# SebastianBitsch/SRGAN-ST

Measured on AMD Instinct MI355X. Metric: HR images/sec (96px x4, B=16/GPU) G+D+ST-loss step, higher is better.
Workload: dtype f32; 1 GPU; srgan_x4_hr96_b16_G+D+ST-loss step: adv+mse+st, D updated every step (train.py:116-164; BASELINE metric); global_batch=16, hr=96, lr=24, parallelism=dp1, hip_graph=True, d_update_interval=1, d_sr_forward=run: all three discriminator forwards of train.py:136,155,158

## Files before the change

### include/srganst.h

```cpp
#ifndef SRGANST_H
#define SRGANST_H
#include <stdint.h>
#ifdef __cplusplus
extern "C" {
#endif

const char* sst_last_error(void);
int sst_version(void);
const char* sst_arch(void);
int sst_clear_error(void);
int sst_reload_env(void);

int sst_st_loss_workspace(int B, int H, int W, int64_t* partial_floats);
int sst_st_loss_fwd(const float* sr, const float* gt, float* loss, float* gS, float* partials,
                    unsigned* counter, int B, int H, int W, float sigma, float rho, int normalize,
                    void* stream);
int sst_st_loss_bwd(const float* sr, const float* gS, float* dsr, const float* scale_dev,
                    float scale_host, int accumulate, int B, int H, int W, float sigma, float rho,
                    void* stream);
int sst_st_maps_workspace(int B, int H, int W, int64_t* tile_floats);
int sst_st_maps(const float* x, const float* gt, float* Sx, float* Sgt, float* Fx, float* Fgt, float* d, float* tile_sums,
                int B, int H, int W, float sigma, float rho, int normalize, void* stream);
int sst_st_pixel_loss_fwd(const float* sr, const float* gt, float* loss, float* gS, float* partials, unsigned* counter,
                          float* pix_loss, float* pix_partials, int pix_mode, int B, int H, int W, float sigma, float rho,
// ... 182 lines not shown
int sst_pixel_loss_fwd(const float* x, const float* gt, float* loss, float* partials, unsigned* counter,
                       int64_t n, int mode, void* stream);
int sst_pixel_loss_bwd(const float* x, const float* gt, float* dx, const float* scale_dev,
                       float scale_host, int accumulate, int64_t n, int mode, void* stream);
int sst_bce_logits(const float* logits, float target, float* loss, float* dlogits,
                   const float* scale_dev, float scale_host, int n, void* stream);
int sst_bicubic(const float* x, float* y, const float* wy, const int* iy, const float* wx, const int* ix,
                int64_t planes, int H, int W, int oh, int ow, int Ty, int Tx, int round_grid, void* stream);
int sst_gather_batch(const uint8_t* src, int64_t N, const int* idx, int B, int H, int W, const float* lut, float* gt, float* lr,
                     const float* wy, const int* iy, const float* wx, const int* ix, int oh, int ow, int Ty, int Tx,
                     void* stream);
int sst_gather_crops(const uint8_t* arena, int64_t arena_bytes, const int64_t* table, int64_t N, const int* desc, int B, int S,
                     const float* lut, float* gt, float* lr, const float* wy, const int* iy, const float* wx, const int* ix,
                     int oh, int ow, int Ty, int Tx, int span, void* stream);
int sst_image_metrics_workspace(int B, int H, int W, int64_t* partial_doubles);
int sst_image_metrics(const float* sr, const float* hr, int B, int H, int W, double* out, uint8_t* sr_u8, uint8_t* hr_u8,
                      double* workspace, void* stream);
int sst_tile_gather(const uint8_t* src_u8, const float* src_f32, int64_t src_bytes, int H, int W, const int* desc, int B, int th,
                    int tw, int t, const float* lut, float* out, void* stream);
int sst_tile_scatter(const float* tiles, const int* rows, int B, int H, int W, int th, int tw, int scale, int t, float* canvas,
                     int accumulate, void* stream);
int sst_canvas_to_u8(const float* canvas, int H, int W, float scale, uint8_t* out, void* stream);
int sst_bb_blocks(int B, int H, int W);
int sst_bb_feature_dim(int mode);
int sst_bb_patches(const float* img, float* cand, float* cnrm, int B, int H, int W, int ncand_total, int cand_off,
                   int mode, const float* st_mats, void* stream);
int sst_bb_match(const float* sr, const float* cand, const float* cnrm, int* ind, float* dsr, float* partials, int B,
                 int H, int W, int ncand, float alpha, float beta, int criterion_l2, int mode, const float* st_mats,
                 void* stream);
int sst_bb_match_dist(const float* sr, const float* cand, const float* cnrm, int* ind, float* dsr, float* partials, int B,
                 int H, int W, int ncand, float alpha, float beta, int criterion_l2, int mode, const float* st_mats, int dist_l1,
                      void* stream);
int sst_bbg_patches(int H, int W, int k, int pad, int stride);
int sst_bbg_blocks(int B, int np);
int sst_bbg_unfold(const float* img, float* table, float* nrm, int B, int H, int W, int k, int pad, int stride, int nrows_total,
                   int row_off, void* stream);
int sst_bbg_match(const float* srf, const float* cand, const float* cnrm, int* ind, float* gfeat, float* partials, int B, int np,
                  int ncand, int D, float alpha, float beta, int criterion_l2, int dist_l1, void* stream);
int sst_bbg_fold(const float* gfeat, float* dsr, int B, int H, int W, int k, int pad, int stride, void* stream);
int sst_weighted_sum(const float* const* terms, const float* weights, int n, float* out, float* weighted,
                     void* stream);

int sst_linear_ksplit(int M, int N, int K);
int sst_linear_fwd(const float* x, const float* w, const float* bias, float* y, float* slab, int M, int N,
                   int K, void* stream);
int sst_linear_dgrad(const float* dy, const float* w, float* dx, int M, int N, int K, int nhwc_C,
                     int nhwc_HW, void* stream);
int sst_linear_wgrad(const float* dy, const float* x, float* dw, float* db, int M, int N, int K,
                     int accumulate, void* stream);
int sst_head_fwd(const float* h, const float* w, const float* b, float* y, int M, int N, int K, float slope,
                 void* stream);
int sst_head_bwd(const float* h, const float* w, const float* dy, float* dh, float* dw, float* db, int M,
                 int N, int K, float slope, int accumulate, void* stream);
int sst_flatten_act(const float* y, const float* scale, const float* shift, float slope, int act,
                    float* flat, int B, int HW, int C, void* stream);
int sst_flatten_act_grp(const float* y, const float* scale, const float* shift, float slope, int act,
                        float* flat, int B, int HW, int C, int grp_images, void* stream);

int sst_adam_flat(float* p, const float* g, float* m, float* v, int64_t n, const float* lr, float* steps,
                  int nsteps, double beta1, double beta2, double eps, double weight_decay, void* stream);

#ifdef __cplusplus
}
#endif
#endif
```

### srgan-st_amd/csrc/linear.hip

```cpp
#include "common.h"

typedef float f32x4 __attribute__((ext_vector_type(4)));

namespace {
constexpr int NT = 256;
constexpr int MAXM = 64;

__global__ __launch_bounds__(NT) void linear_fwd_kernel(const float* __restrict__ x, const float* __restrict__ w,
                                                        float* __restrict__ slab, int M, int N, int K, int kslice) {
  __shared__ float red[4][MAXM][17];
  const int wave = __builtin_amdgcn_readfirstlane(threadIdx.x >> 6), lane = threadIdx.x & 63;
  const int lj = lane & 15, lq = lane >> 4;
  const int n0 = blockIdx.x * 16;
  const int kb = blockIdx.y * kslice, ke = min(K, kb + kslice);
  const int mt = (M + 15) / 16;
  f32x4 acc[4];
#pragma unroll
  for (int t = 0; t < 4; ++t) acc[t] = f32x4{0.f, 0.f, 0.f, 0.f};
  const int n = min(n0 + lj, N - 1);
  const float* wrow = w + (size_t)n * K;
  for (int k = kb + wave * 16; k < ke; k += 64) {
    const int kk = k + 4 * lq;
    f32x4 bv = {0.f, 0.f, 0.f, 0.f};
    if (kk + 3 < ke) {
      bv = *reinterpret_cast<const f32x4*>(wrow + kk);
    } else {
#pragma unroll
      for (int j = 0; j < 4; ++j)
        if (kk + j < ke) bv[j] = wrow[kk + j];
    }
#pragma unroll
    for (int t = 0; t < 4; ++t) {
      if (t < mt) {
        const int m = t * 16 + lj;
        f32x4 av = {0.f, 0.f, 0.f, 0.f};
        if (m < M) {
          if (kk + 3 < ke) {
            av = *reinterpret_cast<const f32x4*>(x + (size_t)m * K + kk);
          } else {
#pragma unroll
            for (int j = 0; j < 4; ++j)
              if (kk + j < ke) av[j] = x[(size_t)m * K + kk + j];
          }
        }
#pragma unroll
        for (int j = 0; j < 4; ++j) acc[t] = __builtin_amdgcn_mfma_f32_16x16x4f32(av[j], bv[j], acc[t], 0, 0, 0);
      }
    }
  }
#pragma unroll
  for (int t = 0; t < 4; ++t)
#pragma unroll
    for (int r = 0; r < 4; ++r) red[wave][t * 16 + 4 * lq + r][lj] = acc[t][r];
  __syncthreads();
  for (int i = threadIdx.x; i < M * 16; i += NT) {
    const int m = i >> 4, j = i & 15;
    if (n0 + j < N)
      slab[((size_t)blockIdx.y * M + m) * N + n0 + j] = red[0][m][j] + red[1][m][j] + red[2][m][j] + red[3][m][j];
  }
}

__global__ __launch_bounds__(NT) void linear_reduce_kernel(const float* __restrict__ slab, const float* __restrict__ bias,
                                                           float* __restrict__ y, int nslab, int M, int N) {
  const int total = M * N;
  for (int i = blockIdx.x * NT + threadIdx.x; i < total; i += gridDim.x * NT) {
    float t = bias ? bias[i % N] : 0.f;
    for (int s = 0; s < nslab; ++s) t += slab[(size_t)s * total + i];
    y[i] = t;
  }
}

template <int MT>
__global__ __launch_bounds__(NT) void linear_dgrad_kernel(const float* __restrict__ dy, const float* __restrict__ w,
                                                          float* __restrict__ dx, int M, int N, int K, int C, int HW) {
  __shared__ float red[4][16][65];
  const int wave = __builtin_amdgcn_readfirstlane(threadIdx.x >> 6), lane = threadIdx.x & 63;
  const int lj = lane & 15, lq = lane >> 4;
  const int k0 = blockIdx.x * 64;
  const int nper = ((N + 3) / 4 + 3) / 4 * 4;
  const int nb = wave * nper, ne = min(N, nb + nper);
  f32x4 acc[MT][4];
#pragma unroll
  for (int mt = 0; mt < MT; ++mt)
#pragma unroll
    for (int t = 0; t < 4; ++t) acc[mt][t] = f32x4{0.f, 0.f, 0.f, 0.f};
  int n = nb;
  if (k0 + 64 <= K) {
    constexpr int U = MT == 1 ? 8 : 4;
    const float* wcol = w + k0 + 4 * lj;
    for (; n + 4 * U <= ne; n += 4 * U) {
      f32x4 bv[U];
      float av[MT][U];
#pragma unroll
      for (int u = 0; u < U; ++u) {
        const int nn = n + 4 * u + lq;
        bv[u] = *reinterpret_cast<const f32x4*>(wcol + (size_t)nn * K);
#pragma unroll
        for (int mt = 0; mt < MT; ++mt) {
          const int m = mt * 16 + lj;
          av[mt][u] = m < M ? dy[(size_t)m * N + nn] : 0.f;
        }
      }
#pragma unroll
      for (int u = 0; u < U; ++u)
#pragma unroll
        for (int mt = 0; mt < MT; ++mt)
#pragma unroll
          for (int t = 0; t < 4; ++t) acc[mt][t] = __builtin_amdgcn_mfma_f32_16x16x4f32(av[mt][u], bv[u][t], acc[mt][t], 0, 0, 0);
    }
  }
  for (; n < ne; n += 4) {
    const int nn = n + lq;
    f32x4 bv = {0.f, 0.f, 0.f, 0.f};
    if (nn < ne) {
      const int kk = k0 + 4 * lj;
      if (kk + 3 < K) {
        bv = *reinterpret_cast<const f32x4*>(w + (size_t)nn * K + kk);
      } else {
#pragma unroll
        for (int j = 0; j < 4; ++j)
          if (kk + j < K) bv[j] = w[(size_t)nn * K + kk + j];
      }
    }
#pragma unroll
    for (int mt = 0; mt < MT; ++mt) {
      const int m = mt * 16 + lj;
      const float av = (nn < ne && m < M) ? dy[(size_t)m * N + nn] : 0.f;
#pragma unroll
      for (int t = 0; t < 4; ++t) acc[mt][t] = __builtin_amdgcn_mfma_f32_16x16x4f32(av, bv[t], acc[mt][t], 0, 0, 0);
    }
  }
#pragma unroll
  for (int mt = 0; mt < MT; ++mt) {
    __syncthreads();
#pragma unroll
    for (int t = 0; t < 4; ++t)
#pragma unroll
      for (int r = 0; r < 4; ++r) red[wave][4 * lq + r][4 * lj + t] = acc[mt][t][r];
    __syncthreads();
    for (int i = threadIdx.x; i < 16 * 64; i += NT) {
      const int mm = i >> 6, kc = i & 63, mg = mt * 16 + mm, k = k0 + kc;
      if (mg < M && k < K) {
        const float v = red[0][mm][kc] + red[1][mm][kc] + red[2][mm][kc] + red[3][mm][kc];
        const size_t o = HW > 0 ? (size_t)mg * K + (size_t)(k % HW) * C + k / HW : (size_t)mg * K + k;
        dx[o] = v;
      }
    }
  }
}

__global__ __launch_bounds__(NT) void linear_wgrad_kernel(const float* __restrict__ dy, const float* __restrict__ x,
                                                          float* __restrict__ dw, int M, int N, int K, int accumulate) {
  __shared__ float sdy[MAXM][16];
  const int n0 = blockIdx.y * 16;
  for (int i = threadIdx.x; i < M * 16; i += NT) {
    const int m = i >> 4, j = i & 15;
    sdy[m][j] = (n0 + j < N) ? dy[(size_t)m * N + n0 + j] : 0.f;
  }
  __syncthreads();
  const int k = (blockIdx.x * NT + threadIdx.x) * 4;
  if (k >= K) return;
  const bool vec = (K & 3) == 0;
  f32x4 acc[16];
#pragma unroll
  for (int j = 0; j < 16; ++j) acc[j] = f32x4{0.f, 0.f, 0.f, 0.f};
  for (int m = 0; m < M; ++m) {
    f32x4 xv = {0.f, 0.f, 0.f, 0.f};
    if (vec) {
      xv = *reinterpret_cast<const f32x4*>(x + (size_t)m * K + k);
    } else {
#pragma unroll
      for (int j = 0; j < 4; ++j)
        if (k + j < K) xv[j] = x[(size_t)m * K + k + j];
    }
#pragma unroll
    for (int j = 0; j < 16; ++j) acc[j] += sdy[m][j] * xv;
  }
#pragma unroll
  for (int j = 0; j < 16; ++j) {
    if (n0 + j >= N) break;
// ... 108 lines not shown
#pragma unroll
          for (int i = 0; i < HB_ROWS; ++i) v[i] = mb + i < M ? h[(size_t)(mb + i) * K + k] : 0.f;
#pragma unroll
          for (int i = 0; i < HB_ROWS; ++i) {
            if (mb + i >= M) break;
            const float x = v[i] > 0.f ? v[i] : v[i] * slope;
            a = fmaf(dy[(size_t)(mb + i) * N + n], x, a);
          }
        }
        dw[(size_t)n * K + k] = accumulate ? dw[(size_t)n * K + k] + a : a;
      }
    }
  }
  if (db && blockIdx.x == 0 && blockIdx.y == 0 && threadIdx.x < N) {
    float t = 0.f;
    for (int m = 0; m < M; ++m) t += dy[(size_t)m * N + threadIdx.x];
    db[threadIdx.x] = accumulate ? db[threadIdx.x] + t : t;
  }
}

__global__ __launch_bounds__(NT) void flatten_act_kernel(const float* __restrict__ y, const float* __restrict__ scale,
                                                         const float* __restrict__ shift, float slope, int act,
                                                         float* __restrict__ flat, int B, int HW, int C, int gB) {
  const int64_t total = (int64_t)B * HW * C;
  for (int64_t i = blockIdx.x * (int64_t)NT + threadIdx.x; i < total; i += (int64_t)gridDim.x * NT) {
    const int c = (int)(i % C);
    const int64_t p = i / C;
    const int hw = (int)(p % HW);
    const int64_t b = p / HW;
    float v = y[i];
    if (scale) {
      const int gc = (int)(b / gB) * C + c;
      v = fmaf(v, scale[gc], shift[gc]);
    }
    if (act) v = v > 0.f ? v : v * slope;
    flat[(b * C + c) * HW + hw] = v;
  }
}
}

SST_API int sst_linear_ksplit(int M, int N, int K) {
  int ks = 1024 / ((N + 15) / 16);
  if (ks < 1) ks = 1;
  while (ks > 1 && K / ks < 256) ks >>= 1;
  return ks;
}

SST_API int sst_linear_fwd(const float* x, const float* w, const float* bias, float* y, float* slab, int M, int N, int K,
                           void* stream) {
  SST_REQUIRE(x && w && y && slab && M > 0 && M <= MAXM && N > 0 && K > 0, "sst_linear_fwd: bad argument (M=%d)", M);
  const int ks = sst_linear_ksplit(M, N, K);
  const int kslice = ((K + ks - 1) / ks + 63) / 64 * 64;
  dim3 grid((N + 15) / 16, (K + kslice - 1) / kslice);
  linear_fwd_kernel<<<grid, NT, 0, sst_stream(stream)>>>(x, w, slab, M, N, K, kslice);
  SST_LAUNCH_CHECK("linear_fwd_kernel");
  const int rb = (M * N + NT - 1) / NT;
  linear_reduce_kernel<<<rb < 512 ? rb : 512, NT, 0, sst_stream(stream)>>>(slab, bias, y, grid.y, M, N);
  SST_LAUNCH_CHECK("linear_reduce_kernel");
  return SST_OK;
}

SST_API int sst_linear_dgrad(const float* dy, const float* w, float* dx, int M, int N, int K, int nhwc_C, int nhwc_HW,
                             void* stream) {
  SST_REQUIRE(dy && w && dx && M > 0 && M <= MAXM && N > 0 && K > 0, "sst_linear_dgrad: bad argument");
  SST_REQUIRE(nhwc_HW == 0 || nhwc_C * nhwc_HW == K, "sst_linear_dgrad: C*HW must equal K");
  const int grid = (K + 63) / 64;
  hipStream_t st = sst_stream(stream);
  switch ((M + 15) / 16) {
    case 1: linear_dgrad_kernel<1><<<grid, NT, 0, st>>>(dy, w, dx, M, N, K, nhwc_C, nhwc_HW); break;
    case 2: linear_dgrad_kernel<2><<<grid, NT, 0, st>>>(dy, w, dx, M, N, K, nhwc_C, nhwc_HW); break;
    case 3: linear_dgrad_kernel<3><<<grid, NT, 0, st>>>(dy, w, dx, M, N, K, nhwc_C, nhwc_HW); break;
    default: linear_dgrad_kernel<4><<<grid, NT, 0, st>>>(dy, w, dx, M, N, K, nhwc_C, nhwc_HW); break;
  }
  SST_LAUNCH_CHECK("linear_dgrad_kernel");
  return SST_OK;
}

SST_API int sst_linear_wgrad(const float* dy, const float* x, float* dw, float* db, int M, int N, int K, int accumulate,
                             void* stream) {
  SST_REQUIRE(dy && x && dw && M > 0 && M <= MAXM && N > 0 && K > 0, "sst_linear_wgrad: bad argument");
  if ((K & 31) == 0 && (N & 63) == 0 && !sst_env("SST_LINEAR_WGRAD_FMA")) {
    linear_wgrad_mfma_kernel<<<dim3((K / 32 + 3) / 4, N / 64), NT, 0, sst_stream(stream)>>>(dy, x, dw, M, N, K, accumulate);
    SST_LAUNCH_CHECK("linear_wgrad_mfma_kernel");
  } else {
    dim3 grid((K + 4 * NT - 1) / (4 * NT), (N + 15) / 16);
    linear_wgrad_kernel<<<grid, NT, 0, sst_stream(stream)>>>(dy, x, dw, M, N, K, accumulate);
    SST_LAUNCH_CHECK("linear_wgrad_kernel");
  }
  if (db) {
    colsum_small_kernel<<<(N + 255) / 256, 256, 0, sst_stream(stream)>>>(dy, db, M, N, accumulate);
    SST_LAUNCH_CHECK("colsum_small_kernel");
  }
  return SST_OK;
}

SST_API int sst_head_fwd(const float* h, const float* w, const float* b, float* y, int M, int N, int K, float slope,
                         void* stream) {
  SST_REQUIRE(h && w && y && M > 0 && N > 0 && N <= 64 && K > 0, "sst_head_fwd: bad argument");
  head_fwd_kernel<<<M * N, NT, 0, sst_stream(stream)>>>(h, w, b, y, M, N, K, slope);
  SST_LAUNCH_CHECK("head_fwd_kernel");
  return SST_OK;
}

SST_API int sst_head_bwd(const float* h, const float* w, const float* dy, float* dh, float* dw, float* db, int M, int N,
                         int K, float slope, int accumulate, void* stream) {
  SST_REQUIRE(h && w && dy && dh && M > 0 && N > 0 && N <= 64 && K > 0, "sst_head_bwd: bad argument");
  head_bwd_kernel<<<dim3((K + NT - 1) / NT, (M + HB_ROWS - 1) / HB_ROWS), NT, 0, sst_stream(stream)>>>(h, w, dy, dh, dw, db, M, N, K, slope,
                                                                                                    accumulate);
  SST_LAUNCH_CHECK("head_bwd_kernel");
  return SST_OK;
}

SST_API int sst_flatten_act_grp(const float* y, const float* scale, const float* shift, float slope, int act, float* flat,
                                int B, int HW, int C, int grp_images, void* stream) {
  SST_REQUIRE(y && flat && B > 0 && HW > 0 && C > 0 && ((scale == nullptr) == (shift == nullptr)), "sst_flatten_act: bad argument");
  SST_REQUIRE(grp_images >= 0 && (grp_images == 0 || B % grp_images == 0), "sst_flatten_act: bad group size %d for B=%d", grp_images, B);
  const int64_t total = (int64_t)B * HW * C;
  const int blocks = (int)((total + NT - 1) / NT < 2048 ? (total + NT - 1) / NT : 2048);
  flatten_act_kernel<<<blocks, NT, 0, sst_stream(stream)>>>(y, scale, shift, slope, act, flat, B, HW, C, grp_images > 0 ? grp_images : B);
  SST_LAUNCH_CHECK("flatten_act_kernel");
  return SST_OK;
}
SST_API int sst_flatten_act(const float* y, const float* scale, const float* shift, float slope, int act, float* flat,
                            int B, int HW, int C, void* stream) {
  return sst_flatten_act_grp(y, scale, shift, slope, act, flat, B, HW, C, 0, stream);
}
// ... 1 lines not shown
```

### srgan-st_amd/srganst/_abi.py

```python
from __future__ import annotations

import ctypes
import os
from ctypes import c_char_p, c_float, c_int, c_int64, c_void_p, POINTER

_HERE = os.path.dirname(os.path.abspath(__file__))
LIB_PATH = os.environ.get("SST_LIB_PATH") or os.path.join(_HERE, "lib", "libsrganst.so")

P = c_void_p

SIGNATURES = {
    "sst_last_error": (c_char_p, []),
    "sst_version": (c_int, []),
    "sst_arch": (c_char_p, []),
    "sst_clear_error": (c_int, []),
    "sst_reload_env": (c_int, []),
    "sst_st_loss_workspace": (c_int, [c_int, c_int, c_int, POINTER(c_int64)]),
    "sst_st_loss_fwd": (c_int, [P, P, P, P, P, P, c_int, c_int, c_int, c_float, c_float, c_int, P]),
    "sst_st_loss_bwd": (c_int, [P, P, P, P, c_float, c_int, c_int, c_int, c_int, c_float, c_float, P]),
    "sst_st_pixel_loss_fwd": (c_int, [P, P, P, P, P, P, P, P, c_int, c_int, c_int, c_int, c_float, c_float, c_int, P]),
    "sst_st_pixel_loss_bwd": (c_int, [P, P, P, P, P, c_float, c_float, c_int, c_int, c_int, c_int, c_int, c_float, c_float, P]),
    "sst_st_maps_workspace": (c_int, [c_int, c_int, c_int, POINTER(c_int64)]),
    "sst_st_maps": (c_int, [P, P, P, P, P, P, P, P, c_int, c_int, c_int, c_float, c_float, c_int, P]),
    "sst_conv_packed_floats": (c_int64, [c_int, c_int, c_int]),
# ... 69 lines not shown
    "sst_transpose": (c_int, [P, P, c_int, c_int, c_int, c_int, c_int, P]),
    "sst_transpose_affine": (c_int, [P, P, c_int, c_int, c_int, c_int, c_int, P, P, P]),
    "sst_maxpool_relu_fwd": (c_int, [P, P, c_int, c_int, c_int, c_int, P]),
    "sst_maxpool_relu_bwd": (c_int, [P, P, P, c_int, c_int, c_int, c_int, P]),
    "sst_clamp_bwd_blocks": (c_int, [c_int, c_int, c_int]),
    "sst_clamp_bwd": (c_int, [P, P, P, P, P, c_int, c_int, c_int, c_int, c_int, P]),
    "sst_pixel_loss_blocks": (c_int, [c_int64]),
    "sst_pixel_loss_fwd": (c_int, [P, P, P, P, P, c_int64, c_int, P]),
    "sst_pixel_loss_bwd": (c_int, [P, P, P, P, c_float, c_int, c_int64, c_int, P]),
    "sst_bce_logits": (c_int, [P, c_float, P, P, P, c_float, c_int, P]),
    "sst_bicubic": (c_int, [P, P, P, P, P, P, c_int64, c_int, c_int, c_int, c_int, c_int, c_int, c_int, P]),
    "sst_gather_batch": (c_int, [P, c_int64, P, c_int, c_int, c_int, P, P, P, P, P, P, P, c_int, c_int, c_int, c_int, P]),
    "sst_gather_crops": (c_int, [P, c_int64, P, c_int64, P, c_int, c_int, P, P, P, P, P, P, P, c_int, c_int, c_int, c_int, c_int, P]),
    "sst_image_metrics_workspace": (c_int, [c_int, c_int, c_int, POINTER(c_int64)]),
    "sst_image_metrics": (c_int, [P, P, c_int, c_int, c_int, P, P, P, P, P]),
    "sst_tile_gather": (c_int, [P, P, c_int64, c_int, c_int, P, c_int, c_int, c_int, c_int, P, P, P]),
    "sst_tile_scatter": (c_int, [P, P, c_int, c_int, c_int, c_int, c_int, c_int, c_int, P, c_int, P]),
    "sst_canvas_to_u8": (c_int, [P, c_int, c_int, c_float, P, P]),
    "sst_feat_loss_fwd": (c_int, [P, P, P, P, c_float, c_int, P, P, P, c_int64, c_int, P]),
    "sst_feat_loss_bwd": (c_int, [P, P, P, P, c_float, c_int, P, P, c_float, c_int, c_int64, c_int, P]),
    "sst_bb_blocks": (c_int, [c_int, c_int, c_int]),
    "sst_bb_feature_dim": (c_int, [c_int]),
    "sst_bb_patches": (c_int, [P, P, P, c_int, c_int, c_int, c_int, c_int, c_int, P, P]),
    "sst_bb_match": (c_int, [P, P, P, P, P, P, c_int, c_int, c_int, c_int, c_float, c_float, c_int, c_int, P, P]),
    "sst_bb_match_dist": (c_int, [P, P, P, P, P, P, c_int, c_int, c_int, c_int, c_float, c_float, c_int, c_int, P, c_int, P]),
    "sst_bbg_patches": (c_int, [c_int, c_int, c_int, c_int, c_int]),
    "sst_bbg_blocks": (c_int, [c_int, c_int]),
    "sst_bbg_unfold": (c_int, [P, P, P, c_int, c_int, c_int, c_int, c_int, c_int, c_int, c_int, P]),
    "sst_bbg_match": (c_int, [P, P, P, P, P, P, c_int, c_int, c_int, c_int, c_float, c_float, c_int, c_int, P]),
    "sst_bbg_fold": (c_int, [P, P, c_int, c_int, c_int, c_int, c_int, c_int, P]),
    "sst_weighted_sum": (c_int, [POINTER(c_void_p), POINTER(c_float), c_int, P, P, P]),
    "sst_wgrad_c3_supported": (c_int, [c_int, c_int]),
    "sst_wgrad_c3_slab_floats": (c_int64, [c_int, c_int, c_int, c_int]),
    "sst_wgrad_c3": (c_int, [P, P, P, P, P, c_float, c_int, c_int, c_int, c_int, c_int, c_int, c_int, P]),
    "sst_conv9_c3_packed_floats": (c_int64, [c_int]),
    "sst_conv9_c3_pack": (c_int, [P, P, c_int, c_int, c_int, P]),
    "sst_conv9_c3_fwd": (c_int, [P, P, P, P, c_int, c_int, c_int, c_int, P]),
    "sst_conv9_to3_packed_floats": (c_int64, [c_int]),
    "sst_conv9_to3_pack": (c_int, [P, P, c_int, P]),
    "sst_conv9_to3_fwd": (c_int, [P, P, P, P, P, P, c_float, c_int, c_int, c_int, c_int, c_int, P]),
    "sst_conv_s2_dgrad_tiles": (c_int, [c_int, c_int, c_int]),
    "sst_conv_s2_dgrad_kernel_name": (c_char_p, [c_int, c_int, c_int, c_int, c_int, c_int]),
    "sst_conv_s2_dgrad_fused": (c_int, [P, P, P, P, P, P, P, P, c_float, c_int, P, P, P, P, P, P, P, c_float, c_int, P,
                                        c_int, c_int, c_int, c_int, c_int, P]),
    "sst_conv_s2_dgrad_packed_floats": (c_int64, [c_int, c_int]),
    "sst_conv_s2_dgrad_pack": (c_int, [P, P, c_int, c_int, P]),
    "sst_conv_s2_dgrad": (c_int, [P, P, P, c_int, c_int, c_int, c_int, c_int, P]),
    "sst_linear_ksplit": (c_int, [c_int, c_int, c_int]),
    "sst_linear_fwd": (c_int, [P, P, P, P, P, c_int, c_int, c_int, P]),
    "sst_linear_dgrad": (c_int, [P, P, P, c_int, c_int, c_int, c_int, c_int, P]),
    "sst_linear_wgrad": (c_int, [P, P, P, P, c_int, c_int, c_int, c_int, P]),
    "sst_head_fwd": (c_int, [P, P, P, P, c_int, c_int, c_int, c_float, P]),
    "sst_head_bwd": (c_int, [P, P, P, P, P, P, c_int, c_int, c_int, c_float, c_int, P]),
    "sst_flatten_act": (c_int, [P, P, P, c_float, c_int, P, c_int, c_int, c_int, P]),
    "sst_flatten_act_grp": (c_int, [P, P, P, c_float, c_int, P, c_int, c_int, c_int, c_int, P]),
}

_lib = None


class HipPathError(RuntimeError):
    pass


def lib() -> ctypes.CDLL:
    global _lib
    if _lib is None:
        if not os.path.exists(LIB_PATH):
            raise HipPathError(
                f"{LIB_PATH} is missing - build it with `python -c 'import __graft_entry__ as g; g.build()'` "
                "(make -C srgan-st_amd/csrc).  There is no CPU fallback for the HIP path.")
        import torch
        l = ctypes.CDLL(LIB_PATH)
        for name, (res, args) in SIGNATURES.items():
            fn = getattr(l, name)
            fn.restype = res
            fn.argtypes = args
        _lib = l
    return _lib


def reload_env() -> None:
    if _lib is not None:
        _lib.sst_reload_env()


def check(rc: int, what: str) -> None:
    if rc != 0:
        msg = lib().sst_last_error().decode(errors="replace")
        raise HipPathError(f"{what} failed (code {rc}): {msg}")


def ptr(t) -> int:
    if t is None:
        return None
    if not t.is_cuda:
        raise HipPathError("HIP path needs tensors on a ROCm device (no CPU fallback)")
    if not t.is_contiguous():
        raise HipPathError("HIP path needs contiguous tensors")
    return t.data_ptr()


def stream_ptr() -> int:
    import torch
    return torch.cuda.current_stream().cuda_stream
```

### srgan-st_amd/srganst/disc_graph.py

```python
from __future__ import annotations

import torch

from . import ops
from ._state import KeptPass, state
from .ops import ACT_SLOPE

LRELU = 0.2


def param_dict(module):
    names = [n for n, _ in module.named_parameters()]
    return names, dict(zip(names, [t.detach() for t in module.parameters()]))


PLAN = [(0, None, 1), (2, 3, 2), (5, 6, 1), (8, 9, 2), (11, 12, 1), (14, 15, 2), (17, 18, 1), (20, 21, 2)]


def _packs(module, p, with_dgrad, counter_add=0):
    hs = state(module)
    cache = hs.cache
    names = [f"features.{ci}.weight" for ci, _, s in PLAN]
    n1 = [f"features.{ci}.weight" for ci, _, s in PLAN if s == 1]
    n2 = [f"features.{ci}.weight" for ci, _, s in PLAN if s == 2]
# ... 127 lines not shown
        rec["scale"], rec["shift"] = scale, shift
        sv["layers"].append(rec)
        h, act = y, ACT_SLOPE
    nfeat = h.shape[1] * h.shape[2] * h.shape[3]
    flat = ops.flatten_act(h, scale, shift, LRELU, 1, grp=gB, out=A("flat", (h.shape[0], nfeat), h))
    h1 = ops.linear_fwd(flat, p["classifier.0.weight"], p["classifier.0.bias"],
                        out=A("h1", (h.shape[0], p["classifier.0.weight"].shape[0]), h))
    if ar is not None:
        ar.filled.add(slot)
    out = ops.head_fwd(h1, p["classifier.2.weight"], p["classifier.2.bias"], LRELU)
    sv["flat"], sv["h1"] = flat, h1
    return out, sv


def replay_running_stats(module, p, sv):
    groups = sv.get("groups", 1)
    if not state(module).counters_external:
        ops.flatten_bn_counters(module).add_(groups)
    for rec in sv["layers"]:
        if rec["bi"] is None:
            continue
        bn = module.features[rec["bi"]]
        ops.bn_finalize(rec["st"], rec["cnt"], p[f"features.{rec['bi']}.weight"], p[f"features.{rec['bi']}.bias"],
                        bn.running_mean, bn.running_var, groups=groups)


def _grad_views(module, p, need_param_grads):
    names = list(p.keys())
    hs = state(module)
    scope = hs.grad_accum if need_param_grads else None
    acc = scope is not None and scope.flat is not None
    if acc:
        plist = [p[n] for n in names]
        offs, _ = ops.flat_layout(plist)
        views = {n: scope.flat[o:o + t.numel()].view(t.shape) for n, t, o in zip(names, plist, offs)}
    else:
        views = ops.flat_grads(module, names, [p[n] for n in names]) if need_param_grads else {}
        if scope is not None:
            scope.flat = hs.flat_grads[-1]
    return views, acc


def backward_classifier(module, p, sv, dout, need_param_grads, st=None):
    views, acc = _grad_views(module, p, need_param_grads)
    grads = {}

    def G(name):
        t = views[name]
        grads[name] = t
        return t

    h1, flat = sv["h1"], sv["flat"]
    wg = need_param_grads
    dh1 = ops.head_bwd(h1, p["classifier.2.weight"], dout.contiguous(), LRELU,
                       dw=G("classifier.2.weight") if wg else None, db=G("classifier.2.bias") if wg else None, accumulate=acc)
    if wg:
        dw0, db0 = G("classifier.0.weight"), G("classifier.0.bias")
        with ops.SideStream(dh1, flat, dw0, db0):
            ops.linear_wgrad(dh1, flat, dw0, db0, accumulate=acc)
    last = sv["layers"][-1]
    B, H, W, C = last["y"].shape
    g = ops.linear_dgrad(dh1, p["classifier.0.weight"], nhwc=(C, H * W)).view(B, H, W, C)
    return {"views": views, "acc": acc, "grads": grads, "g": g}


def backward_features(module, p, sv, st, need_param_grads, need_dx, defer_wgrad=None, defer_below=None):
    views, acc, grads, g = st["views"], st["acc"], st["grads"], st["g"]

    def G(name):
        t = views[name]
        grads[name] = t
        return t

    wg = need_param_grads
    dx = None
    groups, gB = sv.get("groups", 1), sv.get("gB", 0)
    wd, ws2 = sv["wd"], sv["ws2"]
    part = None
    reduces = [] if ops.WGRAD_REDUCE_MULTI else None
    for li in reversed(range(len(sv["layers"]))):
        r = sv["layers"][li]
        y = r["y"]
        n = y.numel() // y.shape[-1] // groups
        ci, bi = r["ci"], r["bi"]
        w = p[f"features.{ci}.weight"]
        if bi is not None:
            gam = p[f"features.{bi}.weight"]
            dg = G(f"features.{bi}.weight") if wg else torch.empty_like(gam)
            db = G(f"features.{bi}.bias") if wg else torch.empty_like(gam)
            kw = dict(scale=r["scale"], shift=r["shift"], slope_const=LRELU, act=1, mean=r["mean"], rstd=r["rstd"], gamma=gam,
                      dgamma=dg, dbeta=db, accumulate=acc and wg, groups=groups)
            dy = ops.bwd_finalize_apply(part, g, y, n, **kw) if part is not None else ops.bwd_reduce_apply(g, y, n, **kw)
        elif wg:
            kw = dict(slope_const=LRELU, act=1, dbeta=G(f"features.{ci}.bias"), accumulate=acc, groups=groups)
            dy = ops.bwd_finalize_apply(part, g, y, n, **kw) if part is not None else ops.bwd_reduce_apply(g, y, n, **kw)
        else:
            dy = ops.bwd_apply(g, y, slope_const=LRELU, act=1, groups=groups)
        part = None
        if wg:
            dwc = G(f"features.{ci}.weight")

            def launch(r=r, dy=dy, dwc=dwc, red=None):
                ops.conv_wgrad(r["x"], dy, dwc, 3, r["stride"], in_scale=r["x_scale"], in_shift=r["x_shift"],
                               in_slope_const=LRELU, in_act=r["x_act"], accumulate=acc, grp=gB, defer_reduce=red)
            if defer_wgrad is not None and (defer_below is None or li < defer_below):
                ev = torch.cuda.Event()
                ev.record()
                defer_wgrad.append((ev, launch, (r["x"], dy, dwc, r["x_scale"], r["x_shift"])))
            else:
                with ops.SideStream(r["x"], dy, dwc):
                    launch(red=reduces)
        if li == 0 and not need_dx:
            break
        xin = r["x"]
# ... 58 lines not shown
```

### srgan-st_amd/srganst/ops.py

```python
from __future__ import annotations

import os

import torch

from . import _abi
from ._abi import check, ptr, stream_ptr
from ._state import state

OUT_NHWC, OUT_SHUFFLE, OUT_NCHW_CLAMP, OUT_UNSHUFFLE = 0, 1, 2, 3
ACT_NONE, ACT_SLOPE = 0, 1
BN_EPS, BN_MOMENTUM = 1e-5, 0.1


PROFILE = None


TRACE = None


def _trace(name, flops, fn, *keep):
    if TRACE is not None:
        TRACE.setdefault(name, []).append((fn, flops, keep))

# ... 489 lines not shown
            (g, y2, cA, cB, cC, in_scale, in_shift, in_slope, dy, wp, dx, epi_y, epi_scale, epi_shift, epi_slope, partial))
    return dx, dy, partial


def linear_fwd(x, w, bias, out=None):
    M, K = x.shape
    N = w.shape[0]
    y = out if out is not None else _f32(M, N, like=x)
    assert tuple(y.shape) == (M, N) and y.is_contiguous()
    slab = _f32(_abi.lib().sst_linear_ksplit(M, N, K) * M * N, like=x)
    args = (ptr(x), ptr(w), ptr(bias), ptr(y), ptr(slab), M, N, K)
    check(_abi.lib().sst_linear_fwd(*args, stream_ptr()), "sst_linear_fwd")
    _trace_hbm("linear_fwd_kernel", 4.0 * (N * K + M * K + M * N), lambda: _abi.lib().sst_linear_fwd(*args, stream_ptr()), x, w, bias, y, slab)
    return y


def linear_dgrad(dy, w, nhwc=None):
    M, N = dy.shape
    K = w.shape[1]
    dx = _f32(M, K, like=dy)
    c, hw = nhwc if nhwc else (0, 0)
    args = (ptr(dy), ptr(w), ptr(dx), M, N, K, c, hw)
    check(_abi.lib().sst_linear_dgrad(*args, stream_ptr()), "sst_linear_dgrad")
    _trace_hbm("linear_dgrad_kernel", 4.0 * (N * K + M * K + M * N), lambda: _abi.lib().sst_linear_dgrad(*args, stream_ptr()), dy, w, dx)
    return dx


def linear_wgrad(dy, x, dw, db=None, accumulate=False):
    M, N = dy.shape
    K = x.shape[1]
    args = (ptr(dy), ptr(x), ptr(dw), ptr(db), M, N, K, int(accumulate))
    check(_abi.lib().sst_linear_wgrad(*args, stream_ptr()), "sst_linear_wgrad")
    _trace_hbm("linear_wgrad_kernel", 4.0 * (N * K * (2 if accumulate else 1) + M * K + M * N),
               lambda: _abi.lib().sst_linear_wgrad(*args, stream_ptr()), dy, x, dw, db)


def head_fwd(h, w, b, slope):
    M, K = h.shape
    N = w.shape[0]
    y = _f32(M, N, like=h)
    check(_abi.lib().sst_head_fwd(ptr(h), ptr(w), ptr(b), ptr(y), M, N, K, float(slope), stream_ptr()), "sst_head_fwd")
    return y


def head_bwd(h, w, dy, slope, dw=None, db=None, accumulate=False):
    M, K = h.shape
    N = w.shape[0]
    dh = torch.empty_like(h)
    check(_abi.lib().sst_head_bwd(ptr(h), ptr(w), ptr(dy), ptr(dh), ptr(dw), ptr(db), M, N, K, float(slope), int(accumulate),
                                  stream_ptr()), "sst_head_bwd")
    return dh


def flatten_act(y, scale, shift, slope, act=1, grp=0, out=None):
    B, H, W, C = y.shape
    flat = out if out is not None else _f32(B, C * H * W, like=y)
    assert tuple(flat.shape) == (B, C * H * W) and flat.is_contiguous()
    check(_abi.lib().sst_flatten_act_grp(ptr(y), ptr(scale), ptr(shift), float(slope), int(act), ptr(flat), B, H * W, C, int(grp),
                                         stream_ptr()), "sst_flatten_act")
    return flat


def wgrad_c3(big, small, dw_out, kind, in_slope=None, in_slope_const=0.0, in_act=ACT_NONE, accumulate=False):
    B, H, W, C = big.shape
    assert tuple(small.shape) == (B, H, W, 3)
    assert tuple(dw_out.shape) == ((3, C, 9, 9) if kind == 0 else (C, 3, 9, 9))
    slab = _f32(_abi.lib().sst_wgrad_c3_slab_floats(B, H, W, C), like=big)
    e0 = _prof_begin()
    check(_abi.lib().sst_wgrad_c3(ptr(big), ptr(small), ptr(slab), ptr(dw_out), ptr(in_slope), float(in_slope_const), int(in_act),
                                  kind, B, H, W, C, int(accumulate), stream_ptr()), "sst_wgrad_c3")
    _prof_end(e0, "wgrad_c3_kernel+reduce", 2.0 * B * H * W * C * 3 * 81)
    return dw_out


def wgrad_c3_supported(C, ksize=9):
    return bool(_abi.lib().sst_wgrad_c3_supported(C, ksize))


PACK_FWD, PACK_DGRAD, PACK_C3_FWD, PACK_C3_DGRAD, PACK_TO3 = 0, 1, 2, 3, 4


class PackPlan:

    def __init__(self, weights, modes, extras=()):
        dev = weights[0].device
        self.ptrs = tuple(w.data_ptr() for w in weights) + self._extras_sig(extras)
        self.out, rows, blk = [], [], 0
        for w, m in zip(weights, modes):
            cout, cin, k, _ = w.shape
            if m == PACK_C3_FWD or m == PACK_C3_DGRAD:
                n = _abi.lib().sst_conv9_c3_packed_floats(cin if m == PACK_C3_DGRAD else cout)
            elif m == PACK_TO3:
                n = _abi.lib().sst_conv9_to3_packed_floats(cin)
            else:
                o, i = (cin, cout) if m else (cout, cin)
                n = _abi.lib().sst_conv_packed_floats(o, i, k)
            assert n < 2 ** 31
            wp = torch.empty(n, device=dev, dtype=torch.float32)
            self.out.append(wp)
            rows.append([w.data_ptr(), wp.data_ptr(), cout | (cin << 32), (k * k) | (int(m) << 32), n, blk])
            blk += (n + 1023) // 1024
        for e in extras:
            if e[0] == "zero":
                t = e[1]
                assert t.is_contiguous() and t.element_size() % 4 == 0
                n = t.numel() * (t.element_size() // 4)
# ... 340 lines not shown
```

Measured before the change: 3261 HR images/s.

## Fuse classifier head backward into linear dgrad and pipeline linear kernels

Adds a classifier_dgrad kernel that computes the LeakyReLU head gradient inline inside the first-linear dgrad when no parameter gradients are needed. This removes a separate head_bwd launch and the dh1 round trip on the discriminator-forward-for-G path. It also templates linear_fwd on the M tile count and batches its loads. The dgrad kernel gets double-buffered load/MFMA batches with sched barriers and launch bounds raised to two blocks. In exchange there are more template instantiations and more register pressure, which could lower occupancy.

```diff
diff --git a/include/srganst.h b/include/srganst.h
--- a/include/srganst.h
+++ b/include/srganst.h
@@ -258,6 +258,8 @@
                  void* stream);
 int sst_head_bwd(const float* h, const float* w, const float* dy, float* dh, float* dw, float* db, int M,
                  int N, int K, float slope, int accumulate, void* stream);
+int sst_classifier_dgrad(const float* h1, const float* w2, const float* dout, const float* w1, float* dx, int M,
+                         int N, int K, float slope, int nhwc_C, int nhwc_HW, void* stream);
 int sst_flatten_act(const float* y, const float* scale, const float* shift, float slope, int act,
                     float* flat, int B, int HW, int C, void* stream);
 int sst_flatten_act_grp(const float* y, const float* scale, const float* shift, float slope, int act,
diff --git a/srgan-st_amd/csrc/linear.hip b/srgan-st_amd/csrc/linear.hip
--- a/srgan-st_amd/csrc/linear.hip
+++ b/srgan-st_amd/csrc/linear.hip
@@ -6,20 +6,44 @@
 constexpr int NT = 256;
 constexpr int MAXM = 64;
 
+template <int MT>
+constexpr int fwd_batch() { return MT == 1 ? 1 : 4; }
+template <int MT>
 __global__ __launch_bounds__(NT) void linear_fwd_kernel(const float* __restrict__ x, const float* __restrict__ w,
                                                         float* __restrict__ slab, int M, int N, int K, int kslice) {
   __shared__ float red[4][MAXM][17];
   const int wave = __builtin_amdgcn_readfirstlane(threadIdx.x >> 6), lane = threadIdx.x & 63;
   const int lj = lane & 15, lq = lane >> 4;
+  constexpr int FWD_U = fwd_batch<MT>();
   const int n0 = blockIdx.x * 16;
   const int kb = blockIdx.y * kslice, ke = min(K, kb + kslice);
-  const int mt = (M + 15) / 16;
-  f32x4 acc[4];
-#pragma unroll
-  for (int t = 0; t < 4; ++t) acc[t] = f32x4{0.f, 0.f, 0.f, 0.f};
+  f32x4 acc[MT];
+#pragma unroll
+  for (int t = 0; t < MT; ++t) acc[t] = f32x4{0.f, 0.f, 0.f, 0.f};
   const int n = min(n0 + lj, N - 1);
   const float* wrow = w + (size_t)n * K;
-  for (int k = kb + wave * 16; k < ke; k += 64) {
+  int k = kb + wave * 16;
+  for (; k + 64 * (FWD_U - 1) + 16 <= ke; k += 64 * FWD_U) {
+    f32x4 bv[FWD_U], av[MT][FWD_U];
+#pragma unroll
+    for (int u = 0; u < FWD_U; ++u) {
+      const int kk = k + 64 * u + 4 * lq;
+      bv[u] = *reinterpret_cast<const f32x4*>(wrow + kk);
+#pragma unroll
+      for (int t = 0; t < MT; ++t) {
+        av[t][u] = *reinterpret_cast<const f32x4*>(x + (size_t)min(t * 16 + lj, M - 1) * K + kk);
+      }
+    }
+    __builtin_amdgcn_sched_barrier(0);
+#pragma unroll
+    for (int u = 0; u < FWD_U; ++u)
+#pragma unroll
+      for (int t = 0; t < MT; ++t)
+#pragma unroll
+        for (int j = 0; j < 4; ++j)
+          acc[t] = __builtin_amdgcn_mfma_f32_16x16x4f32(t * 16 + lj < M ? av[t][u][j] : 0.f, bv[u][j], acc[t], 0, 0, 0);
+  }
+  for (; k < ke; k += 64) {
     const int kk = k + 4 * lq;
     f32x4 bv = {0.f, 0.f, 0.f, 0.f};
     if (kk + 3 < ke) {
@@ -30,26 +54,24 @@
         if (kk + j < ke) bv[j] = wrow[kk + j];
     }
 #pragma unroll
-    for (int t = 0; t < 4; ++t) {
-      if (t < mt) {
-        const int m = t * 16 + lj;
-        f32x4 av = {0.f, 0.f, 0.f, 0.f};
-        if (m < M) {
-          if (kk + 3 < ke) {
-            av = *reinterpret_cast<const f32x4*>(x + (size_t)m * K + kk);
-          } else {
-#pragma unroll
-            for (int j = 0; j < 4; ++j)
-              if (kk + j < ke) av[j] = x[(size_t)m * K + kk + j];
-          }
+    for (int t = 0; t < MT; ++t) {
+      const int m = t * 16 + lj;
+      f32x4 av = {0.f, 0.f, 0.f, 0.f};
+      if (m < M) {
+        if (kk + 3 < ke) {
+          av = *reinterpret_cast<const f32x4*>(x + (size_t)m * K + kk);
+        } else {
+#pragma unroll
+          for (int j = 0; j < 4; ++j)
+            if (kk + j < ke) av[j] = x[(size_t)m * K + kk + j];
         }
-#pragma unroll
-        for (int j = 0; j < 4; ++j) acc[t] = __builtin_amdgcn_mfma_f32_16x16x4f32(av[j], bv[j], acc[t], 0, 0, 0);
-      }
-    }
-  }
-#pragma unroll
-  for (int t = 0; t < 4; ++t)
+      }
+#pragma unroll
+      for (int j = 0; j < 4; ++j) acc[t] = __builtin_amdgcn_mfma_f32_16x16x4f32(av[j], bv[j], acc[t], 0, 0, 0);
+    }
+  }
+#pragma unroll
+  for (int t = 0; t < MT; ++t)
 #pragma unroll
     for (int r = 0; r < 4; ++r) red[wave][t * 16 + 4 * lq + r][lj] = acc[t][r];
   __syncthreads();
@@ -71,7 +93,10 @@
 }
 
 template <int MT>
-__global__ __launch_bounds__(NT) void linear_dgrad_kernel(const float* __restrict__ dy, const float* __restrict__ w,
+constexpr int dgrad_batch() { return MT == 2 ? 8 : 4; }
+template <int MT, bool HEAD>
+__global__ __launch_bounds__(NT, 2) void linear_dgrad_kernel(const float* __restrict__ dy, const float* __restrict__ w2,
+                                                          const float* __restrict__ dout, float slope, const float* __restrict__ w,
                                                           float* __restrict__ dx, int M, int N, int K, int C, int HW) {
   __shared__ float red[4][16][65];
   const int wave = __builtin_amdgcn_readfirstlane(threadIdx.x >> 6), lane = threadIdx.x & 63;
@@ -80,33 +105,69 @@
   const int nper = ((N + 3) / 4 + 3) / 4 * 4;
   const int nb = wave * nper, ne = min(N, nb + nper);
   f32x4 acc[MT][4];
-#pragma unroll
-  for (int mt = 0; mt < MT; ++mt)
+  float dm[MT];
+#pragma unroll
+  for (int mt = 0; mt < MT; ++mt) {
+    dm[mt] = (HEAD && mt * 16 + lj < M) ? dout[mt * 16 + lj] : 0.f;
 #pragma unroll
     for (int t = 0; t < 4; ++t) acc[mt][t] = f32x4{0.f, 0.f, 0.f, 0.f};
+  }
+  auto head_dy = [slope](float hv, float wv, float d) {
+    const float t = fmaf(d, wv, 0.f);
+    return hv > 0.f ? t : t * slope;
+  };
   int n = nb;
   if (k0 + 64 <= K) {
-    constexpr int U = MT == 1 ? 8 : 4;
+    constexpr int U = dgrad_batch<MT>();
     const float* wcol = w + k0 + 4 * lj;
-    for (; n + 4 * U <= ne; n += 4 * U) {
+    struct Batch {
       f32x4 bv[U];
-      float av[MT][U];
+      float av[MT][U], wv[HEAD ? U : 1];
+    };
+    auto load = [&](Batch& b, int n) {
 #pragma unroll
       for (int u = 0; u < U; ++u) {
         const int nn = n + 4 * u + lq;
-        bv[u] = *reinterpret_cast<const f32x4*>(wcol + (size_t)nn * K);
+        b.bv[u] = *reinterpret_cast<const f32x4*>(wcol + (size_t)nn * K);
+        if constexpr (HEAD) b.wv[u] = w2[nn];
 #pragma unroll
         for (int mt = 0; mt < MT; ++mt) {
-          const int m = mt * 16 + lj;
-          av[mt][u] = m < M ? dy[(size_t)m * N + nn] : 0.f;
+          b.av[mt][u] = dy[(size_t)min(mt * 16 + lj, M - 1) * N + nn];
         }
       }
+      __builtin_amdgcn_sched_barrier(0);
+    };
+    auto mma = [&](const Batch& b) {
 #pragma unroll
       for (int u = 0; u < U; ++u)
 #pragma unroll
-        for (int mt = 0; mt < MT; ++mt)
-#pragma unroll
-          for (int t = 0; t < 4; ++t) acc[mt][t] = __builtin_amdgcn_mfma_f32_16x16x4f32(av[mt][u], bv[u][t], acc[mt][t], 0, 0, 0);
+        for (int mt = 0; mt < MT; ++mt) {
+          float a = b.av[mt][u];
+          if constexpr (HEAD) a = head_dy(a, b.wv[u], dm[mt]);
+          if (mt * 16 + lj >= M) a = 0.f;
+#pragma unroll
+          for (int t = 0; t < 4; ++t) acc[mt][t] = __builtin_amdgcn_mfma_f32_16x16x4f32(a, b.bv[u][t], acc[mt][t], 0, 0, 0);
+        }
+      __builtin_amdgcn_sched_barrier(0);
+    };
+    if (n + 4 * U <= ne) {
+      Batch b0, b1;
+      load(b0, n);
+      for (; n + 12 * U <= ne; n += 8 * U) {
+        load(b1, n + 4 * U);
+        mma(b0);
+        load(b0, n + 8 * U);
+        mma(b1);
+      }
+      if (n + 8 * U <= ne) {
+        load(b1, n + 4 * U);
+        mma(b0);
+        mma(b1);
+        n += 8 * U;
+      } else {
+        mma(b0);
+        n += 4 * U;
+      }
     }
   }
   for (; n < ne; n += 4) {
@@ -122,10 +183,12 @@
           if (kk + j < K) bv[j] = w[(size_t)nn * K + kk + j];
       }
     }
+    const float wv = (HEAD && nn < ne) ? w2[nn] : 0.f;
 #pragma unroll
     for (int mt = 0; mt < MT; ++mt) {
       const int m = mt * 16 + lj;
-      const float av = (nn < ne && m < M) ? dy[(size_t)m * N + nn] : 0.f;
+      float av = (nn < ne && m < M) ? dy[(size_t)m * N + nn] : 0.f;
+      if (HEAD) av = (nn < ne && m < M) ? head_dy(av, wv, dm[mt]) : 0.f;
 #pragma unroll
       for (int t = 0; t < 4; ++t) acc[mt][t] = __builtin_amdgcn_mfma_f32_16x16x4f32(av, bv[t], acc[mt][t], 0, 0, 0);
     }
@@ -340,26 +403,48 @@
   const int ks = sst_linear_ksplit(M, N, K);
   const int kslice = ((K + ks - 1) / ks + 63) / 64 * 64;
   dim3 grid((N + 15) / 16, (K + kslice - 1) / kslice);
-  linear_fwd_kernel<<<grid, NT, 0, sst_stream(stream)>>>(x, w, slab, M, N, K, kslice);
+  hipStream_t st = sst_stream(stream);
+  switch ((M + 15) / 16) {
+    case 1: linear_fwd_kernel<1><<<grid, NT, 0, st>>>(x, w, slab, M, N, K, kslice); break;
+    case 2: linear_fwd_kernel<2><<<grid, NT, 0, st>>>(x, w, slab, M, N, K, kslice); break;
+    case 3: linear_fwd_kernel<3><<<grid, NT, 0, st>>>(x, w, slab, M, N, K, kslice); break;
+    default: linear_fwd_kernel<4><<<grid, NT, 0, st>>>(x, w, slab, M, N, K, kslice); break;
+  }
   SST_LAUNCH_CHECK("linear_fwd_kernel");
   const int rb = (M * N + NT - 1) / NT;
-  linear_reduce_kernel<<<rb < 512 ? rb : 512, NT, 0, sst_stream(stream)>>>(slab, bias, y, grid.y, M, N);
+  linear_reduce_kernel<<<rb < 512 ? rb : 512, NT, 0, st>>>(slab, bias, y, grid.y, M, N);
   SST_LAUNCH_CHECK("linear_reduce_kernel");
   return SST_OK;
+}
+
+namespace {
+template <bool HEAD>
+void launch_linear_dgrad(const float* dy, const float* w2, const float* dout, float slope, const float* w, float* dx, int M, int N,
+                         int K, int C, int HW, hipStream_t st) {
+  const int grid = (K + 63) / 64;
+  switch ((M + 15) / 16) {
+    case 1: linear_dgrad_kernel<1, HEAD><<<grid, NT, 0, st>>>(dy, w2, dout, slope, w, dx, M, N, K, C, HW); break;
+    case 2: linear_dgrad_kernel<2, HEAD><<<grid, NT, 0, st>>>(dy, w2, dout, slope, w, dx, M, N, K, C, HW); break;
+    case 3: linear_dgrad_kernel<3, HEAD><<<grid, NT, 0, st>>>(dy, w2, dout, slope, w, dx, M, N, K, C, HW); break;
+    default: linear_dgrad_kernel<4, HEAD><<<grid, NT, 0, st>>>(dy, w2, dout, slope, w, dx, M, N, K, C, HW); break;
+  }
+}
 }
 
 SST_API int sst_linear_dgrad(const float* dy, const float* w, float* dx, int M, int N, int K, int nhwc_C, int nhwc_HW,
                              void* stream) {
   SST_REQUIRE(dy && w && dx && M > 0 && M <= MAXM && N > 0 && K > 0, "sst_linear_dgrad: bad argument");
   SST_REQUIRE(nhwc_HW == 0 || nhwc_C * nhwc_HW == K, "sst_linear_dgrad: C*HW must equal K");
-  const int grid = (K + 63) / 64;
-  hipStream_t st = sst_stream(stream);
-  switch ((M + 15) / 16) {
-    case 1: linear_dgrad_kernel<1><<<grid, NT, 0, st>>>(dy, w, dx, M, N, K, nhwc_C, nhwc_HW); break;
-    case 2: linear_dgrad_kernel<2><<<grid, NT, 0, st>>>(dy, w, dx, M, N, K, nhwc_C, nhwc_HW); break;
-    case 3: linear_dgrad_kernel<3><<<grid, NT, 0, st>>>(dy, w, dx, M, N, K, nhwc_C, nhwc_HW); break;
-    default: linear_dgrad_kernel<4><<<grid, NT, 0, st>>>(dy, w, dx, M, N, K, nhwc_C, nhwc_HW); break;
-  }
+  launch_linear_dgrad<false>(dy, nullptr, nullptr, 0.f, w, dx, M, N, K, nhwc_C, nhwc_HW, sst_stream(stream));
+  SST_LAUNCH_CHECK("linear_dgrad_kernel");
+  return SST_OK;
+}
+
+SST_API int sst_classifier_dgrad(const float* h1, const float* w2, const float* dout, const float* w1, float* dx, int M, int N, int K,
+                                 float slope, int nhwc_C, int nhwc_HW, void* stream) {
+  SST_REQUIRE(h1 && w2 && dout && w1 && dx && M > 0 && M <= MAXM && N > 0 && K > 0, "sst_classifier_dgrad: bad argument");
+  SST_REQUIRE(nhwc_HW == 0 || nhwc_C * nhwc_HW == K, "sst_classifier_dgrad: C*HW must equal K");
+  launch_linear_dgrad<true>(h1, w2, dout, slope, w1, dx, M, N, K, nhwc_C, nhwc_HW, sst_stream(stream));
   SST_LAUNCH_CHECK("linear_dgrad_kernel");
   return SST_OK;
 }
diff --git a/srgan-st_amd/srganst/_abi.py b/srgan-st_amd/srganst/_abi.py
--- a/srgan-st_amd/srganst/_abi.py
+++ b/srgan-st_amd/srganst/_abi.py
@@ -145,6 +145,7 @@
     "sst_linear_wgrad": (c_int, [P, P, P, P, c_int, c_int, c_int, c_int, P]),
     "sst_head_fwd": (c_int, [P, P, P, P, c_int, c_int, c_int, c_float, P]),
     "sst_head_bwd": (c_int, [P, P, P, P, P, P, c_int, c_int, c_int, c_float, c_int, P]),
+    "sst_classifier_dgrad": (c_int, [P, P, P, P, P, c_int, c_int, c_int, c_float, c_int, c_int, P]),
     "sst_flatten_act": (c_int, [P, P, P, c_float, c_int, P, c_int, c_int, c_int, P]),
     "sst_flatten_act_grp": (c_int, [P, P, P, c_float, c_int, P, c_int, c_int, c_int, c_int, P]),
 }
diff --git a/srgan-st_amd/srganst/disc_graph.py b/srgan-st_amd/srganst/disc_graph.py
--- a/srgan-st_amd/srganst/disc_graph.py
+++ b/srgan-st_amd/srganst/disc_graph.py
@@ -203,14 +203,17 @@
 
     h1, flat = sv["h1"], sv["flat"]
     wg = need_param_grads
+    last = sv["layers"][-1]
+    B, H, W, C = last["y"].shape
+    if not wg and p["classifier.2.weight"].shape[0] == 1:
+        g = ops.classifier_dgrad(h1, p["classifier.2.weight"], dout.contiguous(), p["classifier.0.weight"], LRELU, nhwc=(C, H * W))
+        return {"views": views, "acc": acc, "grads": grads, "g": g.view(B, H, W, C)}
     dh1 = ops.head_bwd(h1, p["classifier.2.weight"], dout.contiguous(), LRELU,
                        dw=G("classifier.2.weight") if wg else None, db=G("classifier.2.bias") if wg else None, accumulate=acc)
     if wg:
         dw0, db0 = G("classifier.0.weight"), G("classifier.0.bias")
         with ops.SideStream(dh1, flat, dw0, db0):
             ops.linear_wgrad(dh1, flat, dw0, db0, accumulate=acc)
-    last = sv["layers"][-1]
-    B, H, W, C = last["y"].shape
     g = ops.linear_dgrad(dh1, p["classifier.0.weight"], nhwc=(C, H * W)).view(B, H, W, C)
     return {"views": views, "acc": acc, "grads": grads, "g": g}
 
diff --git a/srgan-st_amd/srganst/ops.py b/srgan-st_amd/srganst/ops.py
--- a/srgan-st_amd/srganst/ops.py
+++ b/srgan-st_amd/srganst/ops.py
@@ -565,6 +565,21 @@
     return dh
 
 
+def classifier_dgrad(h1, w2, dout, w1, slope, nhwc=None):
+    M, N = h1.shape
+    K = w1.shape[1]
+    if w2.shape[0] != 1 or dout.numel() != M:
+        raise _abi.HipPathError(f"classifier_dgrad: the head must have one output (w2 {tuple(w2.shape)}, dout {tuple(dout.shape)})")
+    assert w2.shape[1] == N and w1.shape[0] == N
+    dx = _f32(M, K, like=h1)
+    c, hw = nhwc if nhwc else (0, 0)
+    args = (ptr(h1), ptr(w2), ptr(dout), ptr(w1), ptr(dx), M, N, K, float(slope), c, hw)
+    check(_abi.lib().sst_classifier_dgrad(*args, stream_ptr()), "sst_classifier_dgrad")
+    _trace_hbm("linear_dgrad_kernel", 4.0 * (N * K + M * K + M * N), lambda: _abi.lib().sst_classifier_dgrad(*args, stream_ptr()),
+               h1, w2, dout, w1, dx)
+    return dx
+
+
 def flatten_act(y, scale, shift, slope, act=1, grp=0, out=None):
     B, H, W, C = y.shape
     flat = out if out is not None else _f32(B, C * H * W, like=y)
```

Result: no change. 3254 HR images/s (-0.2%).
